# novara754/arctic-renderer

Measured on AMD Instinct MI355X. Metric: Mshaded-pixels/sec at 4K Sponza, 1 dir + 64 point lights; HBM GB/s vs roofline, higher is better.
Workload: dtype f32

## Files before the change

arctic-renderer_amd/csrc/shade.hip:

```cpp
#include "common.h"
#include "edges.h"
#include "shadow_coords.h"
#include "texture_lod.h"

namespace arctic {

namespace {

typedef const ShadeParams __attribute__((address_space(4))) &SP;
typedef const ShadeParams __attribute__((address_space(4))) *KernArgs;

struct ArgsA { const float4 *ga; const float *gb; uint32_t tiles_x, tiles_y, T, stride; int32_t debug; uint32_t n_materials; };
__device__ __forceinline__ ArgsA args_a(KernArgs a) {
    ArgsA r = {a->g.a, a->g.b, a->tiles_x, a->tiles_y, a->tiles_per_wave, a->group_stride, a->debug, a->n_materials};
    asm volatile("" : "+s"(r.ga), "+s"(r.gb), "+s"(r.tiles_x), "+s"(r.tiles_y), "+s"(r.T), "+s"(r.stride), "+s"(r.debug), "+s"(r.n_materials));
    return r;
}
typedef const uint32_t __attribute__((address_space(4))) *OrderList;
struct OrderArgs { OrderList order; uint32_t n_jobs; };
__device__ __forceinline__ ArgsA args_a_first(KernArgs a, const float *&srgb_lut, const unsigned long long *&vis, OrderArgs &O) {
    ArgsA r = {a->g.a, a->g.b, a->tiles_x, a->tiles_y, a->tiles_per_wave, a->group_stride, a->debug, a->n_materials};
    srgb_lut = a->srgb_lut; vis = a->vis;
    const uint32_t *order = a->tile_order; O.n_jobs = a->n_jobs;
    asm volatile("" : "+s"(r.ga), "+s"(r.gb), "+s"(r.tiles_x), "+s"(r.tiles_y), "+s"(r.T), "+s"(r.stride), "+s"(r.debug), "+s"(r.n_materials), "+s"(srgb_lut), "+s"(vis),
// ... 260 lines not shown
    return shadow / 25.0f;
}


__device__ __forceinline__ bool shadow_table_entry(const ShadowArgs &sa, const ShadowPos &p, uint32_t &offset, bool q8) { return shadow_table_offset(sa.S, sa.pitch, p, offset, q8 ? 4u : 3u); }
__device__ __forceinline__ bool shadow_quick_issue(const ShadowArgs &sa, float lsx, float lsy, float lsz, float lsw, ShadowPos &p, float2 &mm, uint32_t *offset_out = nullptr, bool q8 = false ) {
    mm = make_float2(0.0f, 0.0f);
    if (sa.map == nullptr) return false;
    shadow_coords(lsx, lsy, lsz, lsw, p);
    uint32_t offset = 0;
    const bool in_table = sa.bounds != nullptr && shadow_table_entry(sa, p, offset, q8);
    if (in_table) mm = gload_f2(sa.bounds, offset);
    if (offset_out) *offset_out = offset;
    return in_table;
}
__device__ __forceinline__ bool shadow_quick_decide(const ShadowArgs &sa, bool in_table, const ShadowPos &p, float2 mm, float &lit) {
    lit = 1.0f;
    if (sa.map == nullptr) return true;
    if (in_table) {
        if (p.pz > mm.y) { lit = 0.0f; return true; }
        return !(p.pz > mm.x);
    }
    return p.pz > 1.0f || p.px < 0.0f || p.py < 0.0f || p.px > 1.0f || p.py > 1.0f;
}
__device__ __forceinline__ bool shadow_quick(const ShadowArgs &sa, float lsx, float lsy, float lsz, float lsw, ShadowPos &p, float &lit, bool q8 = false) {
    float2 mm;
    const bool in_table = shadow_quick_issue(sa, lsx, lsy, lsz, lsw, p, mm, nullptr, q8);
    return shadow_quick_decide(sa, in_table, p, mm, lit);
}
__device__ __forceinline__ float shadow_slow(const ShadowArgs &sa, const ShadowPos &p, bool q8 = false ) {
    const uint32_t S = sa.S;
    if (q8) { asm volatile(""); return 1.0f - (S <= 5000u ? shadow_window<true>(sa.map, S, p.px, p.py, p.pz) : shadow_generic(sa.map, S, p.px, p.py, p.pz, true)); }
    return 1.0f - (S <= 5000u ? shadow_window(sa.map, S, p.px, p.py, p.pz) : shadow_generic(sa.map, S, p.px, p.py, p.pz));
}

struct LoopPix {
    f3 n, wo, world;
    float a2, oma2, c4;
    float q2, q1, q0;
};
struct TailPix {
    f3 base;
    float metal, num;
};
struct TailFactors { f3 F0, omF0, kdb; float num; };
__device__ __forceinline__ TailFactors tail_factors(const TailPix &t) {
    TailFactors f;
    f.F0 = mk(fm(t.metal, t.base.x - 0.04f, 0.04f), fm(t.metal, t.base.y - 0.04f, 0.04f), fm(t.metal, t.base.z - 0.04f, 0.04f));
    f.omF0 = mk(1.0f - f.F0.x, 1.0f - f.F0.y, 1.0f - f.F0.z);
    const float km = (1.0f - t.metal) * INV_PI;
    f.kdb = mk(t.base.x * km, t.base.y * km, t.base.z * km);
    f.num = t.num;
    return f;
}
__device__ __forceinline__ void make_pix(f3 n, f3 wo, f3 world, f3 base, float metal, float rough, LoopPix &p, TailPix &t) {
    p.n = n; p.wo = wo; p.world = world;
    t.base = base; t.metal = metal;
    const float ndwo = fmaxf(dot(n, wo), 0.0f);
    const float a = rough * rough, a2 = a * a;
    p.a2 = a2; p.oma2 = 1.0f - a2; p.c4 = -0.25f * p.oma2;
    const float r1 = rough + 1.0f;
    const float k = r1 * r1 * 0.125f, omk = 1.0f - k;
    t.num = a2 * INV_PI * ndwo * rcp(fm(ndwo, omk, k));
    asm volatile("" : "+v"(t.num));
    const float four_ndwo = 4.0f * ndwo;
    p.q2 = omk * four_ndwo; p.q1 = fm(k, four_ndwo, 0.0001f * omk); p.q0 = 0.0001f * k;
}

template <bool POINT>
__device__ __forceinline__ void light_scalars(const LoopPix &p, f3 d, float nd, float &s1, float &s2, float &s3) {
    float inv = 1.0f, inv2 = 1.0f;
    if (POINT) { inv = rsq(dot(d, d)); inv2 = inv * inv; }
    const float ndwi = sat(nd * inv);
    const f3 h = mk(__builtin_fmaf(d.x, inv, p.wo.x), __builtin_fmaf(d.y, inv, p.wo.y), __builtin_fmaf(d.z, inv, p.wo.z));
    const float hh = dot(h, h), rh = rsq(hh);
    const float m = __builtin_fmaf(hh * rh, -0.5f, 1.0f);
    const float m2 = m * m, p5 = m2 * m2 * m;
    const f3 e = mk(__builtin_fmaf(h.x, -rh, p.n.x), __builtin_fmaf(h.y, -rh, p.n.y), __builtin_fmaf(h.z, -rh, p.n.z));
    const float e2 = dot(e, e);
    const float dd = __builtin_fmaf(e2, __builtin_fmaf(e2, p.c4, p.oma2), p.a2);
    const float den = (dd * dd) * __builtin_fmaf(__builtin_fmaf(p.q2, ndwi, p.q1), ndwi, p.q0);
    const float sc = ndwi * inv2;
    s2 = (sc * ndwi) * rcp(den);
    s1 = __builtin_fmaf(-sc, p5, sc);
    s3 = s2 * p5;
}

typedef float v2 __attribute__((ext_vector_type(2)));

#define PK_SEL(H) template <> __device__ __forceinline__
template <int H> __device__ __forceinline__ v2 pk_sub_sb(v2 l, v2 w);
template <int H> __device__ __forceinline__ v2 pk_mul_b(v2 a, v2 b);
template <int H> __device__ __forceinline__ v2 pk_fma_b1(v2 a, v2 b, v2 c);
template <int H> __device__ __forceinline__ v2 pk_fma_b2(v2 a, v2 b, v2 c);
template <int H> __device__ __forceinline__ v2 pk_fnma_b2(v2 a, v2 b, v2 c);
template <int H1, int H2> __device__ __forceinline__ v2 pk_fma_b12(v2 a, v2 b, v2 c);
#define PK_DEFS(H)                                                                                                                          \
    PK_SEL(H) v2 pk_sub_sb<H>(v2 l, v2 w) { v2 r; asm("v_pk_add_f32 %0, %1, %2 op_sel:[0," #H "] op_sel_hi:[1," #H "] neg_lo:[0,1] neg_hi:[0,1]" : "=v"(r) : "s"(l), "v"(w)); return r; } \
    PK_SEL(H) v2 pk_mul_b<H>(v2 a, v2 b) { v2 r; asm("v_pk_mul_f32 %0, %1, %2 op_sel:[0," #H "] op_sel_hi:[1," #H "]" : "=v"(r) : "v"(a), "v"(b)); return r; } \
    PK_SEL(H) v2 pk_fma_b1<H>(v2 a, v2 b, v2 c) { v2 r; asm("v_pk_fma_f32 %0, %1, %2, %3 op_sel:[0," #H ",0] op_sel_hi:[1," #H ",1]" : "=v"(r) : "v"(a), "v"(b), "v"(c)); return r; } \
    PK_SEL(H) v2 pk_fma_b2<H>(v2 a, v2 b, v2 c) { v2 r; asm("v_pk_fma_f32 %0, %1, %2, %3 op_sel:[0,0," #H "] op_sel_hi:[1,1," #H "]" : "=v"(r) : "v"(a), "v"(b), "v"(c)); return r; } \
    PK_SEL(H) v2 pk_fnma_b2<H>(v2 a, v2 b, v2 c) { v2 r; asm("v_pk_fma_f32 %0, %1, %2, %3 op_sel:[0,0," #H "] op_sel_hi:[1,1," #H "] neg_lo:[1,0,0] neg_hi:[1,0,0]" : "=v"(r) : "v"(a), "v"(b), "v"(c)); return r; }
PK_DEFS(0)
PK_DEFS(1)
#define PK_DEFS2(H1, H2)                                                                                                                    \
    template <> __device__ __forceinline__ v2 pk_fma_b12<H1, H2>(v2 a, v2 b, v2 c) { v2 r; asm("v_pk_fma_f32 %0, %1, %2, %3 op_sel:[0," #H1 "," #H2 "] op_sel_hi:[1," #H1 "," #H2 "]" : "=v"(r) : "v"(a), "v"(b), "v"(c)); return r; }
PK_DEFS2(0, 0)
PK_DEFS2(0, 1)
PK_DEFS2(1, 0)
PK_DEFS2(1, 1)
__device__ __forceinline__ v2 pk_fma(v2 a, v2 b, v2 c) { return __builtin_elementwise_fma(a, b, c); }
__device__ __forceinline__ void pk_fma_s(v2 c, v2 s, v2 &acc) { asm("v_pk_fma_f32 %0, %1, %2, %0" : "+v"(acc) : "s"(c), "v"(s)); }
__device__ __forceinline__ v2 pk_mul_sat(v2 a, v2 b) { v2 r; asm("v_pk_mul_f32 %0, %1, %2 clamp" : "=v"(r) : "v"(a), "v"(b)); return r; }
__device__ __forceinline__ v2 rsq2_and_mul_b0(v2 a, v2 x, v2 y, v2 &t) {
    float r0, r1;
    asm("v_rsq_f32 %0, %3\n\tv_rsq_f32 %1, %4\n\tv_pk_mul_f32 %2, %5, %6 op_sel:[0,0] op_sel_hi:[1,0]"
        : "=&v"(r0), "=&v"(r1), "=&v"(t) : "v"(a.x), "v"(a.y), "v"(x), "v"(y));
    return (v2){r0, r1};
}
__device__ __forceinline__ v2 rsq2_and_fma_b01(v2 a, v2 x, v2 y, v2 &t) {
    float r0, r1;
    asm("v_rsq_f32 %0, %3\n\tv_rsq_f32 %1, %4\n\tv_pk_fma_f32 %2, %5, %6, %6 op_sel:[0,0,1] op_sel_hi:[1,0,1]"
        : "=&v"(r0), "=&v"(r1), "=&v"(t) : "v"(a.x), "v"(a.y), "v"(x), "v"(y));
    return (v2){r0, r1};
}
__device__ __forceinline__ v2 rcp2_and_mul(v2 a, v2 x, v2 y, v2 &t) {
    float r0, r1;
    asm("v_rcp_f32 %0, %3\n\tv_rcp_f32 %1, %4\n\tv_pk_mul_f32 %2, %5, %6"
        : "=&v"(r0), "=&v"(r1), "=&v"(t) : "v"(a.x), "v"(a.y), "v"(x), "v"(y));
    return (v2){r0, r1};
}

struct Sums { float a[3], b[3], c[3]; };
struct Sums2 { v2 a[3], b[3], c[3]; };
__device__ __forceinline__ f3 resolve_sums(const TailPix &tp, const float A[3], const float B[3], const float C[3]) {
    const TailFactors t = tail_factors(tp);
    return mk(fm(t.kdb.x * t.omF0.x, A[0], t.num * fm(t.F0.x, B[0], t.omF0.x * C[0])),
              fm(t.kdb.y * t.omF0.y, A[1], t.num * fm(t.F0.y, B[1], t.omF0.y * C[1])),
              fm(t.kdb.z * t.omF0.z, A[2], t.num * fm(t.F0.z, B[2], t.omF0.z * C[2])));
}

struct PackedPix { v2 n_xy, nz_wox, wo_yz, w_xy, wz_a2, oma2_c4, q21, q0_; };
__device__ __forceinline__ PackedPix pack_pix(const LoopPix &p) {
    PackedPix k;
    k.n_xy = (v2){p.n.x, p.n.y}; k.nz_wox = (v2){p.n.z, p.wo.x}; k.wo_yz = (v2){p.wo.y, p.wo.z};
    k.w_xy = (v2){p.world.x, p.world.y}; k.wz_a2 = (v2){p.world.z, p.a2}; k.oma2_c4 = (v2){p.oma2, p.c4};
    k.q21 = (v2){p.q2, p.q1}; k.q0_ = (v2){p.q0, 0.0f};
    return k;
}
typedef float f4v __attribute__((ext_vector_type(4)));
__device__ __forceinline__ void load_light_pair(const char *p , f4v &A, f4v &B, f4v &C) {
    asm volatile("s_load_dwordx4 %0, %3, 0x0\n\ts_load_dwordx4 %1, %3, 0x10\n\ts_load_dwordx4 %2, %3, 0x20" : "=&s"(A), "=&s"(B), "=&s"(C) : "s"(p));
}
__device__ __forceinline__ void wait_and_sub(v2 lx, v2 ly, v2 lz, v2 w_xy, v2 wz, v2 &dx, v2 &dy, v2 &dz) {
    asm volatile("s_waitcnt lgkmcnt(0)\n\t"
                 "v_pk_add_f32 %0, %3, %6 op_sel:[0,0] op_sel_hi:[1,0] neg_lo:[0,1] neg_hi:[0,1]\n\t"
                 "v_pk_add_f32 %1, %4, %6 op_sel:[0,1] op_sel_hi:[1,1] neg_lo:[0,1] neg_hi:[0,1]\n\t"
                 "v_pk_add_f32 %2, %5, %7 op_sel:[0,0] op_sel_hi:[1,0] neg_lo:[0,1] neg_hi:[0,1]"
                 : "=&v"(dx), "=&v"(dy), "=&v"(dz) : "s"(lx), "s"(ly), "s"(lz), "v"(w_xy), "v"(wz));
}

__device__ __forceinline__ v2 accumulate_pair(const PackedPix &k, v2 dx, v2 dy, v2 dz, v2 cr, v2 cg, v2 cb, Sums2 &S) {
    const v2 d2 = pk_fma(dz, dz, pk_fma(dy, dy, dx * dx));
    v2 ndx;
    const v2 inv = rsq2_and_mul_b0(d2, dx, k.n_xy, ndx);
    const v2 nd = pk_fma_b1<0>(dz, k.nz_wox, pk_fma_b1<1>(dy, k.n_xy, ndx));
    const v2 ndwi = pk_mul_sat(nd, inv);
    const v2 hx = pk_fma_b2<1>(dx, inv, k.nz_wox), hy = pk_fma_b2<0>(dy, inv, k.wo_yz), hz = pk_fma_b2<1>(dz, inv, k.wo_yz);
    const v2 hh = pk_fma(hz, hz, pk_fma(hy, hy, hx * hx));
    v2 q;
    const v2 rh = rsq2_and_fma_b01(hh, ndwi, k.q21, q);
    const v2 m = pk_fma(hh * rh, (v2){-0.5f, -0.5f}, (v2){1.0f, 1.0f});
    const v2 ex = pk_fnma_b2<0>(hx, rh, k.n_xy), ey = pk_fnma_b2<1>(hy, rh, k.n_xy), ez = pk_fnma_b2<0>(hz, rh, k.nz_wox);
    const v2 e2 = pk_fma(ez, ez, pk_fma(ey, ey, ex * ex));
    const v2 dd = pk_fma_b2<1>(e2, pk_fma_b12<1, 0>(e2, k.oma2_c4, k.oma2_c4), k.wz_a2);
    const v2 den = (dd * dd) * pk_fma_b2<0>(q, ndwi, k.q0_);
    const v2 sc = ndwi * (inv * inv);
    v2 m2;
    const v2 rden = rcp2_and_mul(den, m, m, m2);
    const v2 p5 = m2 * m2 * m;
    const v2 s2 = (sc * ndwi) * rden;
    const v2 s1 = pk_fma(-sc, p5, sc), s3 = s2 * p5;
    pk_fma_s(cr, s1, S.a[0]); pk_fma_s(cg, s1, S.a[1]); pk_fma_s(cb, s1, S.a[2]);
    pk_fma_s(cr, s2, S.b[0]); pk_fma_s(cg, s2, S.b[1]); pk_fma_s(cb, s2, S.b[2]);
    pk_fma_s(cr, s3, S.c[0]); pk_fma_s(cg, s3, S.c[1]); pk_fma_s(cb, s3, S.c[2]);
    return nd;
}

__device__ __forceinline__ float rrt_odt(float c) {
    float a = fm(c, c + 0.0245786f, -0.000090537f);
    float b = fm(c, fm(0.983729f, c, 0.4329510f), 0.238081f);
    return a * rcp(b);
}
__device__ __forceinline__ v2 pk_fma_sat(v2 k , v2 a, v2 c) { v2 r; asm("v_pk_fma_f32 %0, %1, %2, %3 clamp" : "=v"(r) : "s"(k), "v"(a), "v"(c)); return r; }
__device__ __forceinline__ float fma_sat(float k , float a, float c) { float r; asm("v_fma_f32 %0, %1, %2, %3 clamp" : "=v"(r) : "s"(k), "v"(a), "v"(c)); return r; }
__device__ __forceinline__ f3 tonemap(f3 c, int tm, float exposure) {
    f3 t;
    if (tm == 1) {
        const float LOG2E = 1.4426950408889634f;
        const f3 x = mk(c.x * exposure, c.y * exposure, c.z * exposure);
        auto one_minus_exp = [&](float v) {
            const float direct = 1.0f - __builtin_amdgcn_exp2f(-v * LOG2E);
            const float series = v * fm(v, fm(v, 1.0f / 6.0f, -0.5f), 1.0f);
            return fabsf(v) < 0.015625f ? series : direct;
        };
        t = mk(one_minus_exp(x.x), one_minus_exp(x.y), one_minus_exp(x.z));
    } else if (tm == 2) {
        auto pfm = [](v2 a, v2 b, v2 c2) { return __builtin_elementwise_fma(a, b, c2); };
        const v2 cx = {c.x, c.x}, cy = {c.y, c.y}, cz = {c.z, c.z};
        v2 ixy = pfm((v2){0.04823f, 0.01566f}, cz, pfm((v2){0.35458f, 0.90834f}, cy, (v2){0.59719f, 0.07600f} * cx));
        float iz = fm(0.837f, c.z, fm(0.13383f, c.y, 0.02840f * c.x));
        {
            const v2 a = pfm(ixy, ixy + (v2){0.0245786f, 0.0245786f}, (v2){-0.000090537f, -0.000090537f});
            const v2 b = pfm(ixy, pfm((v2){0.983729f, 0.983729f}, ixy, (v2){0.4329510f, 0.4329510f}), (v2){0.238081f, 0.238081f});
            ixy = a * (v2){rcp(b.x), rcp(b.y)};
            iz = rrt_odt(iz);
        }
        const v2 ix = {ixy.x, ixy.x}, iy = {ixy.y, ixy.y}, izz = {iz, iz};
        const v2 oxy = pk_fma_sat((v2){-0.07367f, -0.00605f}, izz, pfm((v2){-0.53108f, 1.10813f}, iy, (v2){1.60475f, -0.10208f} * ix));
        t = mk(oxy.x, oxy.y, fma_sat(1.07f, iz, fm(-0.07276f, ixy.y, -0.00327f * ixy.x)));
    } else {
        t = mk(c.x * rcp(c.x + 1.0f), c.y * rcp(c.y + 1.0f), c.z * rcp(c.z + 1.0f));
    }
    return t;
}
__device__ __forceinline__ f3 gamma_exponent(f3 t, float inv_gamma) {
    return mk(inv_gamma * __builtin_amdgcn_logf(fabsf(t.x)), inv_gamma * __builtin_amdgcn_logf(fabsf(t.y)), inv_gamma * __builtin_amdgcn_logf(fabsf(t.z)));
}
__device__ __forceinline__ f3 post_process(f3 c, int tm, float inv_gamma, float exposure) {
    const f3 g = gamma_exponent(tonemap(c, tm, exposure), inv_gamma);
    return mk(__builtin_amdgcn_exp2f(g.x), __builtin_amdgcn_exp2f(g.y), __builtin_amdgcn_exp2f(g.z));
}
__device__ __forceinline__ uint32_t unorm8(float x) { return (uint32_t)__builtin_fmaf(sat(x), 255.0f, 0.5f); }
__device__ __forceinline__ uint32_t rgba8_word(f3 l) { return unorm8(l.x) | (unorm8(l.y) << 8) | (unorm8(l.z) << 16) | 0xFF000000u; }
__device__ __forceinline__ uint32_t rgba8_word_of_exponents(f3 g) {
    float e0, e1, e2, q0, q1, q2;
    asm("v_exp_f32_e64 %0, %6 clamp\n\tv_exp_f32_e64 %1, %7 clamp\n\tv_exp_f32_e64 %2, %8 clamp\n\t"
        "v_fma_f32 %3, %0, %9, 0.5\n\tv_fma_f32 %4, %1, %9, 0.5\n\tv_fma_f32 %5, %2, %9, 0.5"
        : "=&v"(e0), "=&v"(e1), "=&v"(e2), "=&v"(q0), "=&v"(q1), "=&v"(q2) : "v"(g.x), "v"(g.y), "v"(g.z), "s"(255.0f));
    return (uint32_t)q0 | ((uint32_t)q1 << 8) | ((uint32_t)q2 << 16) | 0xFF000000u;
}

struct TileHead { float4 a; float b0, b1, b2; };
typedef float f3v __attribute__((ext_vector_type(3), aligned(4)));
typedef float f4a __attribute__((ext_vector_type(4)));
__device__ __forceinline__ float4 gload_f4(const void *base, uint32_t o) { const f4a v = *(const f4a __attribute__((address_space(1))) *)((gchar)base + o); return make_float4(v.x, v.y, v.z, v.w); }
__device__ __forceinline__ TileHead load_head(const float4 *ga, const float *gb, size_t tile , uint32_t lane) {
    TileHead t;
    t.a = gload_f4(ga + tile * 64, lane * 16u);
    const f3v b = *(const f3v __attribute__((address_space(1))) *)((gchar)(gb + tile * 192) + lane * 12u);
    t.b0 = b.x; t.b1 = b.y; t.b2 = b.z;
    return t;
}

__device__ __forceinline__ float through_half(float x) { return (float)(_Float16)x; }

__device__ __forceinline__ void store_pixel(const StoreArgs &sa, const uint8_t *out, uint32_t o, uint32_t po, f3 color) {
    if (sa.hdr16) { asm volatile(""); color = mk(through_half(color.x), through_half(color.y), through_half(color.z)); }
    uint32_t word;
    f3 g = mk(0.0f, 0.0f, 0.0f);
    if (sa.debug & 4) { asm volatile(""); word = rgba8_word(color); }
    else {
        g = gamma_exponent(tonemap(color, sa.tm, sa.exposure), sa.inv_gamma);
        word = rgba8_word_of_exponents(g);
    }
    *(uint32_t __attribute__((address_space(1))) *)((char __attribute__((address_space(1))) *)out + o * 4u) = word;
    if (sa.out_ldr) {
        asm volatile("");
        const f3 l = (sa.debug & 4) ? color : mk(__builtin_amdgcn_exp2f(g.x), __builtin_amdgcn_exp2f(g.y), __builtin_amdgcn_exp2f(g.z));
        sa.out_ldr[(size_t)po * 3] = l.x; sa.out_ldr[(size_t)po * 3 + 1] = l.y; sa.out_ldr[(size_t)po * 3 + 2] = l.z;
    }
    if (sa.out_hdr) { asm volatile(""); sa.out_hdr[(size_t)po * 3] = color.x; sa.out_hdr[(size_t)po * 3 + 1] = color.y; sa.out_hdr[(size_t)po * 3 + 2] = color.z; }
}

__device__ __forceinline__ void wrap_axis64(double u, uint32_t n, int &i0, int &i1, float &f) {
    const double uw = u - floor(u);
    const double x = uw * (double)n - 0.5;
    const double xf = floor(x);
    f = (float)(x - xf);
    i0 = (int)xf;
    i1 = i0 + 1;
    if (i0 < 0) i0 += (int)n;
    if (i1 >= (int)n) i1 -= (int)n;
}
__device__ __noinline__ f3 sample_environment(const float4 *__restrict__ env, uint32_t w, uint32_t h, float fx_, float fy_, float fz_) {
    double x = fx_, y = fy_, z = fz_;
    const double inv = 1.0 / sqrt(x * x + y * y + z * z);
    x *= inv; y *= inv; z *= inv;
    const double u = atan2(z, x) * (double)0.1591f + 0.5;
    const double v = -(asin(fmin(fmax(y, -1.0), 1.0)) * (double)0.3183f + 0.5);
    int x0, x1, y0, y1;
    float fx, fy;
    wrap_axis64(u, w, x0, x1, fx);
    wrap_axis64(v, h, y0, y1, fy);
    const float4 a = env[(size_t)y0 * w + x0], b = env[(size_t)y0 * w + x1], c = env[(size_t)y1 * w + x0], d = env[(size_t)y1 * w + x1];
    const float gx = 1.0f - fx, gy = 1.0f - fy;
    const float w00 = gx * gy, w10 = fx * gy, w01 = gx * fy, w11 = fx * fy;
    return mk(fm(w11, d.x, fm(w01, c.x, fm(w10, b.x, w00 * a.x))), fm(w11, d.y, fm(w01, c.y, fm(w10, b.y, w00 * a.y))),
              fm(w11, d.z, fm(w01, c.z, fm(w10, b.z, w00 * a.z))));
}

__device__ __forceinline__ f3 get_normal(float nr, float ng, float nb, const float4 &gc, const float4 &gd, const float4 &ge) {
    const float r = snorm_of_bytes(nr), g = -snorm_of_bytes(ng), b = snorm_of_bytes(nb);
    return normalize(mk(fm(ge.y, b, fm(gd.z, g, gc.w * r)), fm(ge.z, b, fm(gd.w, g, gd.x * r)), fm(ge.w, b, fm(ge.x, g, gd.y * r))));
}
__device__ __forceinline__ void spot_sums(SP sp, const LoopPix &px, float A[3], float B[3], float C[3]) {
    const uint32_t n_spots = sp.n_spots;
    typedef const f4v __attribute__((address_space(4))) *const_f4;
    const const_f4 L = (const_f4)sp.spots;
    const bool cull = sp.culling != 0;
    for (uint32_t i = 0; i < n_spots; ++i) {
        const f4v a = L[SPOT_F4 * i], b = L[SPOT_F4 * i + 1], c = L[SPOT_F4 * i + 2];
        const f3 dl = mk(a.x, a.y, a.z) - px.world;
        const float ndl = dot(px.n, dl);
        const float d2 = dot(dl, dl), inv = rsq(d2);
        const float cd = -dot(mk(b.x, b.y, b.z), dl) * inv;
        const float att = sat(fm(cd, a.w, b.w)), q = d2 * c.w;
        const float f = (att * att) * sat(1.0f - q * q);
        if (cull && __ballot(ndl > 0.0f && f > 0.0f) == 0ull) continue;
        const float cr = c.x * f, cg = c.y * f, cb = c.z * f;
        float s1, s2, s3;
        light_scalars<true>(px, dl, ndl, s1, s2, s3);
        A[0] = __builtin_fmaf(cr, s1, A[0]); A[1] = __builtin_fmaf(cg, s1, A[1]); A[2] = __builtin_fmaf(cb, s1, A[2]);
        B[0] = __builtin_fmaf(cr, s2, B[0]); B[1] = __builtin_fmaf(cg, s2, B[1]); B[2] = __builtin_fmaf(cb, s2, B[2]);
        C[0] = __builtin_fmaf(cr, s3, C[0]); C[1] = __builtin_fmaf(cg, s3, C[1]); C[2] = __builtin_fmaf(cb, s3, C[2]);
    }
}
__device__ __forceinline__ float cube_visibility(const float *faces , uint32_t F, f3 d ,
                                                 float pz_scale, float zn) {
    const float ax = fabsf(d.x), ay = fabsf(d.y), az = fabsf(d.z);
    float m, sd, ud;
    uint32_t face;
    if (ax >= ay && ax >= az) { m = ax; face = d.x >= 0.0f ? 0u : 1u; sd = d.x >= 0.0f ? -d.z : d.z; ud = -d.y; }
    else if (ay >= az) { m = ay; face = d.y >= 0.0f ? 2u : 3u; sd = d.x; ud = d.y >= 0.0f ? d.z : -d.z; }
    else { m = az; face = d.z >= 0.0f ? 4u : 5u; sd = d.z >= 0.0f ? d.x : -d.x; ud = -d.y; }
    if (!(m > zn)) return 1.0f;
    const float im = 1.0f / m;
    const float pz = pz_scale * (1.0f - zn * im);
    if (pz > 1.0f) return 1.0f;
    const float hf = 0.5f * (float)F;
    const float x = __builtin_fmaf(sd * im, hf, hf - 0.5f), y = __builtin_fmaf(-(ud * im), hf, hf - 0.5f);
    const float x0 = floorf(x), y0 = floorf(y);
    const float fx = x - x0, fy = y - y0;
    const int32_t last = (int32_t)F - 1, ix = (int32_t)x0, iy = (int32_t)y0;
    const uint32_t c0 = (uint32_t)min(max(ix, 0), last), c1 = (uint32_t)min(max(ix + 1, 0), last);
    const uint32_t r0 = (uint32_t)min(max(iy, 0), last) * F, r1 = (uint32_t)min(max(iy + 1, 0), last) * F;
    const uint32_t base = face * F * F;
    const float t00 = __uint_as_float(gload_u32(faces, (base + r0 + c0) * 4u)), t10 = __uint_as_float(gload_u32(faces, (base + r0 + c1) * 4u));
    const float t01 = __uint_as_float(gload_u32(faces, (base + r1 + c0) * 4u)), t11 = __uint_as_float(gload_u32(faces, (base + r1 + c1) * 4u));
    const float s00 = pz > t00 ? 1.0f : 0.0f, s10 = pz > t10 ? 1.0f : 0.0f, s01 = pz > t01 ? 1.0f : 0.0f, s11 = pz > t11 ? 1.0f : 0.0f;
    return 1.0f - lerp_exact(lerp_exact(s00, s10, fx), lerp_exact(s01, s11, fx), fy);
}
__device__ __forceinline__ void cube_sums(SP sp, const LoopPix &px, float A[3], float B[3], float C[3]) {
    const uint32_t n_cubes = sp.n_cubes, F = sp.cube_size;
    typedef const f4v __attribute__((address_space(4))) *const_f4;
    const const_f4 L = (const_f4)sp.cubes;
    const float *faces = reinterpret_cast<const float *>(sp.cubes + CUBE_F4 * n_cubes);
    const bool cull = sp.culling != 0;
    for (uint32_t i = 0; i < n_cubes; ++i) {
        const f4v a = L[CUBE_F4 * i], c = L[CUBE_F4 * i + 1];
        const f3 dl = mk(a.x, a.y, a.z) - px.world;
        const float ndl = dot(px.n, dl);
        const bool front = ndl > 0.0f;
        float v = 1.0f;
        if (front) v = cube_visibility(faces + (size_t)i * 6 * F * F, F, mk(-dl.x, -dl.y, -dl.z), a.w, c.w);
        if (cull) {
            if (__ballot(front && v > 0.0f) == 0ull) continue;
            if (!front || v == 0.0f) continue;
        }
        const float cr = c.x * v, cg = c.y * v, cb = c.z * v;
        float s1, s2, s3;
        light_scalars<true>(px, dl, ndl, s1, s2, s3);
        A[0] = __builtin_fmaf(cr, s1, A[0]); A[1] = __builtin_fmaf(cg, s1, A[1]); A[2] = __builtin_fmaf(cb, s1, A[2]);
        B[0] = __builtin_fmaf(cr, s2, B[0]); B[1] = __builtin_fmaf(cg, s2, B[1]); B[2] = __builtin_fmaf(cb, s2, B[2]);
        C[0] = __builtin_fmaf(cr, s3, C[0]); C[1] = __builtin_fmaf(cg, s3, C[1]); C[2] = __builtin_fmaf(cb, s3, C[2]);
    }
}
template <int LOOP, bool STATS, bool SPOT = false, bool CUBE = false>
__device__ __forceinline__ f3 lit_radiance(SP sp, uint32_t lane, float nr, float ng, float nb, float rough, float metal, f3 base,
                                           const float4 &gc, const float4 &gd, const float4 &ge) {
    const f3 n = get_normal(nr, ng, nb, gc, gd, ge);
    const f3 world = mk(gc.x, gc.y, gc.z);
    const LightArgs la = light_args(sp);
    const f3 wo = normalize(mk(la.eye[0], la.eye[1], la.eye[2]) - world);
    asm volatile("" : "+v"(metal));
    LoopPix px;
    TailPix tp;
    make_pix(n, wo, world, base, metal, rough, px, tp);
    unsigned long long contributing = 0ull, wave_zero = 0ull;
    f3 Lo;
    if (LOOP == 1) {
        Sums S;
        {
            const SunArgs sun = sun_args(sp);
            const f3 d = mk(-sun.dir[0], -sun.dir[1], -sun.dir[2]);
            float s1, s2, s3;
            light_scalars<false>(px, d, dot(n, d), s1, s2, s3);
            for (int k = 0; k < 3; ++k) { S.a[k] = sun.color[k] * s1; S.b[k] = sun.color[k] * s2; S.c[k] = sun.color[k] * s3; }
        }
        for (uint32_t i = 0; i < la.n_lights; ++i) {
            typedef const f4v __attribute__((address_space(4))) *const_f4;
            const f4v lp = ((const_f4)la.lights)[2 * i], lc = ((const_f4)la.lights)[2 * i + 1];
            const f3 dl = mk(lp.x, lp.y, lp.z) - world;
            const float ndl = dot(n, dl);
            if (STATS) { const unsigned long long mk_ = __ballot(ndl > 0.0f); contributing += __popcll(mk_); wave_zero += mk_ == 0ull ? 1 : 0; }
            if (sp.culling && ndl <= 0.0f) continue;
            float s1, s2, s3;
            light_scalars<true>(px, dl, ndl, s1, s2, s3);
            S.a[0] = __builtin_fmaf(lc.x, s1, S.a[0]); S.a[1] = __builtin_fmaf(lc.y, s1, S.a[1]); S.a[2] = __builtin_fmaf(lc.z, s1, S.a[2]);
            S.b[0] = __builtin_fmaf(lc.x, s2, S.b[0]); S.b[1] = __builtin_fmaf(lc.y, s2, S.b[1]); S.b[2] = __builtin_fmaf(lc.z, s2, S.b[2]);
            S.c[0] = __builtin_fmaf(lc.x, s3, S.c[0]); S.c[1] = __builtin_fmaf(lc.y, s3, S.c[1]); S.c[2] = __builtin_fmaf(lc.z, s3, S.c[2]);
        }
        if (SPOT) spot_sums(sp, px, S.a, S.b, S.c);
        if (CUBE) cube_sums(sp, px, S.a, S.b, S.c);
        Lo = resolve_sums(tp, S.a, S.b, S.c);
    } else {
        Sums2 S;
        for (int k = 0; k < 3; ++k) { S.a[k] = (v2){0.0f, 0.0f}; S.b[k] = (v2){0.0f, 0.0f}; S.c[k] = (v2){0.0f, 0.0f}; }
        const uint32_t n_pairs = (la.n_lights + 1) >> 1;
        const PackedPix pk = pack_pix(px);
        const char *lp = reinterpret_cast<const char *>(la.pairs);
        auto finish = [&](v2 dx, v2 dy, v2 dz, const f4v &Bq, const f4v &C, uint32_t p) {
            const v2 nd = accumulate_pair(pk, dx, dy, dz, (v2){Bq.z, Bq.w}, (v2){C.x, C.y}, (v2){C.z, C.w}, S);
            if (STATS) {
                const bool second = 2 * p + 1 < la.n_lights;
                const unsigned long long m0 = __ballot(nd.x > 0.0f), m1 = second ? __ballot(nd.y > 0.0f) : ~0ull;
                contributing += __popcll(m0) + (second ? __popcll(m1) : 0);
                wave_zero += (m0 == 0ull ? 1 : 0) + (m1 == 0ull ? 1 : 0);
            }
        };
        if (n_pairs) {
            f4v A0, B0, C0, A1, B1, C1;
            v2 dx, dy, dz;
            load_light_pair(lp, A0, B0, C0);
            for (uint32_t p = 0;;) {
                wait_and_sub((v2){A0.x, A0.y}, (v2){A0.z, A0.w}, (v2){B0.x, B0.y}, pk.w_xy, pk.wz_a2, dx, dy, dz);
                if (p + 1 < n_pairs) load_light_pair(lp + 48 * (p + 1), A1, B1, C1);
                finish(dx, dy, dz, B0, C0, p);
                if (++p == n_pairs) break;
                wait_and_sub((v2){A1.x, A1.y}, (v2){A1.z, A1.w}, (v2){B1.x, B1.y}, pk.w_xy, pk.wz_a2, dx, dy, dz);
                if (p + 1 < n_pairs) load_light_pair(lp + 48 * (p + 1), A0, B0, C0);
                finish(dx, dy, dz, B1, C1, p);
                if (++p == n_pairs) break;
            }
            asm volatile("s_waitcnt lgkmcnt(0)");
        }
        float A[3], Bs[3], Cs[3];
        {
            const SunArgs sun = sun_args(sp);
            const f3 d = mk(-sun.dir[0], -sun.dir[1], -sun.dir[2]);
            float s1, s2, s3;
            light_scalars<false>(px, d, dot(n, d), s1, s2, s3);
            for (int k = 0; k < 3; ++k) {
                A[k] = __builtin_fmaf(sun.color[k], s1, S.a[k].x + S.a[k].y);
                Bs[k] = __builtin_fmaf(sun.color[k], s2, S.b[k].x + S.b[k].y);
                Cs[k] = __builtin_fmaf(sun.color[k], s3, S.c[k].x + S.c[k].y);
            }
        }
        if (SPOT) spot_sums(sp, px, A, Bs, Cs);
        if (CUBE) cube_sums(sp, px, A, Bs, Cs);
        Lo = resolve_sums(tp, A, Bs, Cs);
    }
    if (STATS) {
        const unsigned long long active = __ballot(1);
        if (lane == (uint32_t)__ffsll((long long)active) - 1) {
            atomicAdd(sp.stats, (unsigned long long)__popcll(active) * la.n_lights);
            atomicAdd(sp.stats + 1, (unsigned long long)__popcll(active));
            atomicAdd(sp.stats + 2, contributing);
            atomicAdd(sp.stats + 3, wave_zero);
            atomicAdd(sp.stats + 4, 1ull);
        }
    }
    return Lo;
}

__device__ __forceinline__ f3 env_level(const EnvTables *T, uint32_t k, float u, float v) {
    const float4 *img = T->level[k];
    const uint32_t w = T->w[k], h = T->h[k];
    int x0, x1, y0, y1;
    float fx, fy;
    wrap_axis(u, w, x0, x1, fx);
    wrap_axis(v, h, y0, y1, fy);
    const float4 a = img[(size_t)y0 * w + x0], b = img[(size_t)y0 * w + x1], c = img[(size_t)y1 * w + x0], d = img[(size_t)y1 * w + x1];
    const float gx = 1.0f - fx, gy = 1.0f - fy;
    const float w00 = gx * gy, w10 = fx * gy, w01 = gx * fy, w11 = fx * fy;
    return mk(fm(w11, d.x, fm(w01, c.x, fm(w10, b.x, w00 * a.x))), fm(w11, d.y, fm(w01, c.y, fm(w10, b.y, w00 * a.y))),
              fm(w11, d.z, fm(w01, c.z, fm(w10, b.z, w00 * a.z))));
}
__device__ __forceinline__ f3 env_ambient(const EnvTables *T, f3 n, f3 wo, f3 base, float metal, float rough) {
    typedef const float __attribute__((address_space(4))) *const_f;
    const const_f sh = (const_f)T->sh;
    const float Y[9] = {0.28209479f, 0.48860251f * n.y, 0.48860251f * n.z, 0.48860251f * n.x, 1.09254843f * (n.x * n.y), 1.09254843f * (n.y * n.z),
                        0.31539157f * (3.0f * (n.z * n.z) - 1.0f), 1.09254843f * (n.x * n.z), 0.54627422f * (n.x * n.x - n.y * n.y)};
    float E[3];
#pragma unroll
    for (int c = 0; c < 3; ++c) {
        float e = sh[c] * Y[0];
#pragma unroll
        for (int k = 1; k < 9; ++k) e = fm(sh[3 * k + c], Y[k], e);
        E[c] = e;
    }
    const float ndwo_raw = dot(n, wo), ndwo = fmaxf(ndwo_raw, 0.0f);
    const f3 F0 = mk(fm(metal, base.x - 0.04f, 0.04f), fm(metal, base.y - 0.04f, 0.04f), fm(metal, base.z - 0.04f, 0.04f));
    const float om = 1.0f - ndwo, om2 = om * om, p5 = om2 * om2 * om, omr = 1.0f - rough, oml = 1.0f - metal;
    const f3 F = mk(fm(fmaxf(omr, F0.x) - F0.x, p5, F0.x), fm(fmaxf(omr, F0.y) - F0.y, p5, F0.y), fm(fmaxf(omr, F0.z) - F0.z, p5, F0.z));
    const float lx = fminf(fmaxf(ndwo * (float)ENV_LUT - 0.5f, 0.0f), (float)(ENV_LUT - 1)), ly = fminf(fmaxf(rough * (float)ENV_LUT - 0.5f, 0.0f), (float)(ENV_LUT - 1));
    const uint32_t i0 = (uint32_t)lx, j0 = (uint32_t)ly, i1 = min(i0 + 1u, ENV_LUT - 1), j1 = min(j0 + 1u, ENV_LUT - 1);
    const float ax = lx - (float)i0, ay = ly - (float)j0;
    const float2 l00 = T->lut[j0 * ENV_LUT + i0], l10 = T->lut[j0 * ENV_LUT + i1], l01 = T->lut[j1 * ENV_LUT + i0], l11 = T->lut[j1 * ENV_LUT + i1];
    const float bx = 1.0f - ax, by = 1.0f - ay;
    const float A = fm(ax * ay, l11.x, fm(bx * ay, l01.x, fm(ax * by, l10.x, (bx * by) * l00.x)));
    const float B = fm(ax * ay, l11.y, fm(bx * ay, l01.y, fm(ax * by, l10.y, (bx * by) * l00.y)));
    const float two = 2.0f * ndwo_raw;
    const f3 R = normalize(mk(fm(two, n.x, -wo.x), fm(two, n.y, -wo.y), fm(two, n.z, -wo.z)));
    const float u = atan2f(R.z, R.x) * 0.1591f + 0.5f;
    const float v = -(asinf(fminf(fmaxf(R.y, -1.0f), 1.0f)) * 0.3183f + 0.5f);
    const float t = rough * (float)(ENV_LEVELS - 1);
    const uint32_t k0 = min((uint32_t)t, ENV_LEVELS - 1), k1 = min(k0 + 1u, ENV_LEVELS - 1);
    const float f = t - (float)k0;
    const f3 P0 = env_level(T, k0, u, v), P1 = env_level(T, k1, u, v);
    const f3 P = mk(fm(f, P1.x - P0.x, P0.x), fm(f, P1.y - P0.y, P0.y), fm(f, P1.z - P0.z, P0.z));
    const float kb = oml * INV_PI;
    return mk(fm((1.0f - F.x) * kb * base.x, E[0], P.x * fm(F0.x, A, B)),
              fm((1.0f - F.y) * kb * base.y, E[1], P.y * fm(F0.y, A, B)),
              fm((1.0f - F.z) * kb * base.z, E[2], P.z * fm(F0.z, A, B)));
}

template <int LOOP, bool STATS, class Second>
__device__ __forceinline__ bool shade_tile_fast(SP sp, KernArgs args, const ArgsA &A, const float *lut, uint32_t ty, uint32_t tx, uint32_t lane, const TileHead &cur, Second second) {
    ArgsB B = args_b(args);
    const int32_t row0 = (int32_t)(ty * 8) - (int32_t)B.row0_in_tile;
    if ((A.debug & (1 | 2 | 4 | 256)) != 0 || tx * 8 + 8 > B.width || row0 < 0 || row0 + 8 > (int32_t)B.rows) return false;
    if (B.sh.map != nullptr && B.sh.bounds == nullptr) return false;
    const uint32_t mat = __float_as_uint(cur.b2);
    const uint32_t m0 = __builtin_amdgcn_readfirstlane(mat);
    if (m0 >= A.n_materials || __ballot(mat != m0) != 0ull) return false;
    u8v dv;
    float lsx = cur.a.z;
    tex_desc_issue(B.tex, m0 * 3, dv, lsx);
    ShadowPos spos;
    float2 mm;
    uint32_t toff = 0;
    const bool q8s = (A.debug & SAMPLER_Q8_SHADOW) != 0;
    const bool in_table = shadow_quick_issue(B.sh, lsx, cur.a.w, cur.b0, cur.b1, spos, mm, &toff, q8s);
    TexS d0 = tex_desc_wait(dv, toff);
    if (!d0.packed) return false;
    Taps pt;
    fetch_taps_packed(d0, cur.a.x, cur.a.y, pt, (A.debug & SAMPLER_Q8_MATERIAL) != 0);
    ArgsC C = args_c(args, A, B);
    float lit;
    const bool decided = shadow_quick_decide(B.sh, in_table, spos, mm, lit);
    if (__ballot(!decided) != 0ull) {
        if (B.sh.S > 5000u) return false;
        asm("" : "=v"(pt.r0.x), "=v"(pt.r0.y), "=v"(pt.r0.z), "=v"(pt.r0.w), "=v"(pt.r1.x), "=v"(pt.r1.y), "=v"(pt.r1.z), "=v"(pt.r1.w));
        asm("" : "=v"(pt.w00), "=v"(pt.w10), "=v"(pt.w01), "=v"(pt.w11));
        bool tapped = false;
        if (q8s) { asm volatile(""); if (!decided) lit = 1.0f - shadow_window<true>(B.sh.map, B.sh.S, spos.px, spos.py, spos.pz); }
        else if (!decided) lit = 1.0f - shadow_window(B.sh.map, B.sh.S, spos.px, spos.py, spos.pz, STATS ? &tapped : nullptr);
        if (STATS) {
            const unsigned long long und = __ballot(!decided), tap = __ballot(tapped);
            if (wave_lane() == 0) {
                atomicAdd(sp.stats + 5, 1ull); atomicAdd(sp.stats + 6, (unsigned long long)__popcll(und));
                if (tap) { atomicAdd(sp.stats + 7, 1ull); atomicAdd(sp.stats + 8, (unsigned long long)__popcll(tap)); }
            }
        }
        asm volatile("" : "+s"(args));
        B = args_b(args);
        C = args_c(args, A, B);
        d0 = tex_desc(B.tex, m0 * 3);
        fetch_taps_packed(d0, cur.a.x, cur.a.y, pt, (A.debug & SAMPLER_Q8_MATERIAL) != 0);
    }
    const bool live = B.culling ? lit != 0.0f : true;
    float4 gc, gd, ge;
    if (live) second(C.gc, C.gd, C.ge, gc, gd, ge);
    f3 base = mk(filt_srgb<0>(pt, lut), filt_srgb<1>(pt, lut), filt_srgb<2>(pt, lut));
    asm volatile("" : "+v"(gc.x), "+v"(gc.y), "+v"(gc.z), "+v"(gc.w), "+v"(gd.x), "+v"(gd.y), "+v"(gd.z), "+v"(gd.w), "+v"(ge.x), "+v"(ge.y), "+v"(ge.z), "+v"(ge.w), "+v"(base.x));
    EpiArgs E = {C.st, B.out, B.width, B.row0_in_tile, C.ambient};
    f3 color;
    if (__ballot(live) != 0ull) {
        if (live) {
            const f3 Lo = lit_radiance<LOOP, STATS>(sp, lane, filt_bytes<0, 3>(pt), filt_bytes<1, 0>(pt), filt_bytes<1, 1>(pt),
                                                    filt_unorm<1, 2>(pt), filt_unorm<1, 3>(pt),
                                                    base, gc, gd, ge);
            color = Lo;
        }
        asm volatile("" : "+s"(args));
        E = epi_args(args);
        const f3 amb = base * E.ambient;
        if (live) color = mk(__builtin_fmaf(color.x, lit, amb.x), __builtin_fmaf(color.y, lit, amb.y), __builtin_fmaf(color.z, lit, amb.z));
        else color = amb;
    } else color = base * E.ambient;
    const uint32_t e_width = __builtin_amdgcn_readfirstlane(E.width), e_row0 = __builtin_amdgcn_readfirstlane(E.row0_in_tile);
    const uint32_t tile_px = (ty * 8 - e_row0) * e_width + tx * 8;
    const uint32_t l2 = wave_lane();
    const uint32_t o = __umul24(l2 >> 3, e_width) + (l2 & 7u);
    store_pixel(E.st, E.out + (size_t)tile_px * 4u, o, tile_px + o, color);
    return true;
}
// ... 551 lines not shown
```

Baseline: 44250.

## Software-pipeline light-pair loop, interleaving accumulation with next pair's head math

Restructures the per-pixel point-light loop into a software pipeline. The colour sums for pair p are interleaved in hand-written inline asm with the distance, rsqrt and N·L work for pair p+1, and the colours are saved to SGPRs before the next scalar load overwrites them. This removes the double-buffered A0/A1 register sets and is meant to hide ALU latency and the scalar load wait by giving the scheduler independent work. It adds a lot of fragile inline asm with fixed instruction ordering, which can raise SGPR pressure and block compiler scheduling.

Result: no change. 43970 (-0.6%).

```diff
diff --git a/arctic-renderer_amd/csrc/shade.hip b/arctic-renderer_amd/csrc/shade.hip
--- a/arctic-renderer_amd/csrc/shade.hip
+++ b/arctic-renderer_amd/csrc/shade.hip
@@ -436,6 +436,10 @@
 __device__ __forceinline__ void load_light_pair(const char *p , f4v &A, f4v &B, f4v &C) {
     asm volatile("s_load_dwordx4 %0, %3, 0x0\n\ts_load_dwordx4 %1, %3, 0x10\n\ts_load_dwordx4 %2, %3, 0x20" : "=&s"(A), "=&s"(B), "=&s"(C) : "s"(p));
 }
+__device__ __forceinline__ void keep_colours_and_load_light_pair(const char *p , f4v &A, f4v &B, f4v &C, v2 &cr, v2 &cg, v2 &cb, v2 &pin) {
+    asm volatile("s_mov_b64 %0, %3\n\ts_mov_b64 %1, %4\n\ts_mov_b64 %2, %5" : "=&s"(cr), "=&s"(cg), "=&s"(cb) : "s"((v2){B.z, B.w}), "s"((v2){C.x, C.y}), "s"((v2){C.z, C.w}));
+    asm volatile("s_load_dwordx4 %0, %4, 0x0\n\ts_load_dwordx4 %1, %4, 0x10\n\ts_load_dwordx4 %2, %4, 0x20" : "=&s"(A), "=&s"(B), "=&s"(C), "+v"(pin) : "s"(p));
+}
 __device__ __forceinline__ void wait_and_sub(v2 lx, v2 ly, v2 lz, v2 w_xy, v2 wz, v2 &dx, v2 &dy, v2 &dz) {
     asm volatile("s_waitcnt lgkmcnt(0)\n\t"
                  "v_pk_add_f32 %0, %3, %6 op_sel:[0,0] op_sel_hi:[1,0] neg_lo:[0,1] neg_hi:[0,1]\n\t"
@@ -444,12 +448,20 @@
                  : "=&v"(dx), "=&v"(dy), "=&v"(dz) : "s"(lx), "s"(ly), "s"(lz), "v"(w_xy), "v"(wz));
 }
 
-__device__ __forceinline__ v2 accumulate_pair(const PackedPix &k, v2 dx, v2 dy, v2 dz, v2 cr, v2 cg, v2 cb, Sums2 &S) {
-    const v2 d2 = pk_fma(dz, dz, pk_fma(dy, dy, dx * dx));
+struct PairHead { v2 dx, dy, dz, inv, ndwi, nd; };
+struct PairScalars { v2 s1, s2, s3; };
+__device__ __forceinline__ PairHead pair_head(v2 lx, v2 ly, v2 lz, const PackedPix &k) {
+    PairHead h;
+    wait_and_sub(lx, ly, lz, k.w_xy, k.wz_a2, h.dx, h.dy, h.dz);
+    const v2 d2 = pk_fma(h.dz, h.dz, pk_fma(h.dy, h.dy, h.dx * h.dx));
     v2 ndx;
-    const v2 inv = rsq2_and_mul_b0(d2, dx, k.n_xy, ndx);
-    const v2 nd = pk_fma_b1<0>(dz, k.nz_wox, pk_fma_b1<1>(dy, k.n_xy, ndx));
-    const v2 ndwi = pk_mul_sat(nd, inv);
+    h.inv = rsq2_and_mul_b0(d2, h.dx, k.n_xy, ndx);
+    h.nd = pk_fma_b1<0>(h.dz, k.nz_wox, pk_fma_b1<1>(h.dy, k.n_xy, ndx));
+    h.ndwi = pk_mul_sat(h.nd, h.inv);
+    return h;
+}
+__device__ __forceinline__ PairScalars pair_scalars(const PackedPix &k, const PairHead &h) {
+    const v2 dx = h.dx, dy = h.dy, dz = h.dz, inv = h.inv, ndwi = h.ndwi;
     const v2 hx = pk_fma_b2<1>(dx, inv, k.nz_wox), hy = pk_fma_b2<0>(dy, inv, k.wo_yz), hz = pk_fma_b2<1>(dz, inv, k.wo_yz);
     const v2 hh = pk_fma(hz, hz, pk_fma(hy, hy, hx * hx));
     v2 q;
@@ -463,12 +475,49 @@
     v2 m2;
     const v2 rden = rcp2_and_mul(den, m, m, m2);
     const v2 p5 = m2 * m2 * m;
-    const v2 s2 = (sc * ndwi) * rden;
-    const v2 s1 = pk_fma(-sc, p5, sc), s3 = s2 * p5;
-    pk_fma_s(cr, s1, S.a[0]); pk_fma_s(cg, s1, S.a[1]); pk_fma_s(cb, s1, S.a[2]);
-    pk_fma_s(cr, s2, S.b[0]); pk_fma_s(cg, s2, S.b[1]); pk_fma_s(cb, s2, S.b[2]);
-    pk_fma_s(cr, s3, S.c[0]); pk_fma_s(cg, s3, S.c[1]); pk_fma_s(cb, s3, S.c[2]);
-    return nd;
+    PairScalars s;
+    s.s2 = (sc * ndwi) * rden;
+    s.s1 = pk_fma(-sc, p5, sc); s.s3 = s.s2 * p5;
+    return s;
+}
+__device__ __forceinline__ void pair_sums(v2 cr, v2 cg, v2 cb, const PairScalars &s, Sums2 &S) {
+    pk_fma_s(cr, s.s1, S.a[0]); pk_fma_s(cg, s.s1, S.a[1]); pk_fma_s(cb, s.s1, S.a[2]);
+    pk_fma_s(cr, s.s2, S.b[0]); pk_fma_s(cg, s.s2, S.b[1]); pk_fma_s(cb, s.s2, S.b[2]);
+    pk_fma_s(cr, s.s3, S.c[0]); pk_fma_s(cg, s.s3, S.c[1]); pk_fma_s(cb, s.s3, S.c[2]);
+}
+__device__ __forceinline__ PairHead sums_and_next_head(v2 cr, v2 cg, v2 cb, const PairScalars &s, Sums2 &S, v2 lx, v2 ly, v2 lz, const PackedPix &k) {
+    PairHead h;
+    v2 d2;
+    float r0, r1;
+    asm volatile("s_waitcnt lgkmcnt(0)\n\t"
+                 "v_pk_add_f32 %0, %8, %11 op_sel:[0,0] op_sel_hi:[1,0] neg_lo:[0,1] neg_hi:[0,1]\n\t"
+                 "v_pk_add_f32 %1, %9, %11 op_sel:[0,1] op_sel_hi:[1,1] neg_lo:[0,1] neg_hi:[0,1]\n\t"
+                 "v_pk_add_f32 %2, %10, %12 op_sel:[0,0] op_sel_hi:[1,0] neg_lo:[0,1] neg_hi:[0,1]\n\t"
+                 "v_pk_mul_f32 %3, %0, %0\n\t"
+                 "v_pk_fma_f32 %4, %13, %16, %4\n\t"
+                 "v_pk_fma_f32 %3, %1, %1, %3\n\t"
+                 "v_pk_fma_f32 %5, %14, %16, %5\n\t"
+                 "v_pk_fma_f32 %3, %2, %2, %3\n\t"
+                 "v_pk_fma_f32 %6, %15, %16, %6\n\t"
+                 "v_pk_fma_f32 %7, %13, %17, %7"
+                 : "=&v"(h.dx), "=&v"(h.dy), "=&v"(h.dz), "=&v"(d2), "+v"(S.a[0]), "+v"(S.a[1]), "+v"(S.a[2]), "+v"(S.b[0])
+                 : "s"(lx), "s"(ly), "s"(lz), "v"(k.w_xy), "v"(k.wz_a2), "s"(cr), "s"(cg), "s"(cb), "v"(s.s1), "v"(s.s2));
+    asm volatile("v_rsq_f32 %0, %7\n\t"
+                 "v_rsq_f32 %1, %8\n\t"
+                 "v_pk_mul_f32 %2, %9, %12 op_sel:[0,0] op_sel_hi:[1,0]\n\t"
+                 "v_pk_fma_f32 %3, %15, %17, %3\n\t"
+                 "v_pk_fma_f32 %2, %10, %12, %2 op_sel:[0,1,0] op_sel_hi:[1,1,1]\n\t"
+                 "v_pk_fma_f32 %4, %16, %17, %4\n\t"
+                 "v_pk_fma_f32 %2, %11, %13, %2 op_sel:[0,0,0] op_sel_hi:[1,0,1]\n\t"
+                 "v_pk_fma_f32 %5, %14, %18, %5\n\t"
+                 "v_pk_fma_f32 %6, %15, %18, %6"
+                 : "=&v"(r0), "=&v"(r1), "=&v"(h.nd), "+v"(S.b[1]), "+v"(S.b[2]), "+v"(S.c[0]), "+v"(S.c[1])
+                 : "v"(d2.x), "v"(d2.y), "v"(h.dx), "v"(h.dy), "v"(h.dz), "v"(k.n_xy), "v"(k.nz_wox), "s"(cr), "s"(cg), "s"(cb), "v"(s.s2), "v"(s.s3));
+    h.inv = (v2){r0, r1};
+    asm volatile("v_pk_mul_f32 %0, %2, %3 clamp\n\t"
+                 "v_pk_fma_f32 %1, %4, %5, %1"
+                 : "=v"(h.ndwi), "+v"(S.c[2]) : "v"(h.nd), "v"(h.inv), "s"(cb), "v"(s.s3));
+    return h;
 }
 
 __device__ __forceinline__ float rrt_odt(float c) {
@@ -704,8 +753,7 @@
         const uint32_t n_pairs = (la.n_lights + 1) >> 1;
         const PackedPix pk = pack_pix(px);
         const char *lp = reinterpret_cast<const char *>(la.pairs);
-        auto finish = [&](v2 dx, v2 dy, v2 dz, const f4v &Bq, const f4v &C, uint32_t p) {
-            const v2 nd = accumulate_pair(pk, dx, dy, dz, (v2){Bq.z, Bq.w}, (v2){C.x, C.y}, (v2){C.z, C.w}, S);
+        auto count = [&](v2 nd, uint32_t p) {
             if (STATS) {
                 const bool second = 2 * p + 1 < la.n_lights;
                 const unsigned long long m0 = __ballot(nd.x > 0.0f), m1 = second ? __ballot(nd.y > 0.0f) : ~0ull;
@@ -714,20 +762,19 @@
             }
         };
         if (n_pairs) {
-            f4v A0, B0, C0, A1, B1, C1;
-            v2 dx, dy, dz;
-            load_light_pair(lp, A0, B0, C0);
-            for (uint32_t p = 0;;) {
-                wait_and_sub((v2){A0.x, A0.y}, (v2){A0.z, A0.w}, (v2){B0.x, B0.y}, pk.w_xy, pk.wz_a2, dx, dy, dz);
-                if (p + 1 < n_pairs) load_light_pair(lp + 48 * (p + 1), A1, B1, C1);
-                finish(dx, dy, dz, B0, C0, p);
-                if (++p == n_pairs) break;
-                wait_and_sub((v2){A1.x, A1.y}, (v2){A1.z, A1.w}, (v2){B1.x, B1.y}, pk.w_xy, pk.wz_a2, dx, dy, dz);
-                if (p + 1 < n_pairs) load_light_pair(lp + 48 * (p + 1), A0, B0, C0);
-                finish(dx, dy, dz, B1, C1, p);
-                if (++p == n_pairs) break;
+            f4v A, B, C;
+            load_light_pair(lp, A, B, C);
+            PairHead h = pair_head((v2){A.x, A.y}, (v2){A.z, A.w}, (v2){B.x, B.y}, pk);
+            count(h.nd, 0);
+            for (uint32_t p = 1; p < n_pairs; ++p) {
+                v2 cr, cg, cb;
+                keep_colours_and_load_light_pair(lp + 48 * p, A, B, C, cr, cg, cb, h.inv);
+                const PairScalars s = pair_scalars(pk, h);
+                h = sums_and_next_head(cr, cg, cb, s, S, (v2){A.x, A.y}, (v2){A.z, A.w}, (v2){B.x, B.y}, pk);
+                count(h.nd, p);
             }
-            asm volatile("s_waitcnt lgkmcnt(0)");
+            const PairScalars s = pair_scalars(pk, h);
+            pair_sums((v2){B.z, B.w}, (v2){C.x, C.y}, (v2){C.z, C.w}, s, S);
         }
         float A[3], Bs[3], Cs[3];
         {
```
